# Krist-Marrakesh/Hybrid-Hotel-Recommendation-System-Based-on-Friends-Recommendations

Measured on AMD Instinct MI355X. Metric: fwd+bwd samples/sec (DCN-R train step) + scored (user,hotel) pairs/sec, higher is better.
Workload: dtype bf16; 1 GPU; DCN-R train step: fwd (train BN, dropout 0.6) + BCE + bwd + AdamW (+grad all-reduce), BASELINE configs[2]/[3]; batch_per_gpu=131072, global_batch=131072, tables=1M x 32 users, 100k x 32 hotels, 12 x 1000 x 32 cat, 8 dense, deep=3 cross + 4 x 512 residual, parallelism=dp1, exchange=none

## Files before the change

hybrid-hotel-recommendation-system-based-on-friends-recommendations_amd/csrc/dcnr_api.hip:

```cpp
#include "dcnr_internal.h"

#include <algorithm>
#include <cmath>
#include <cstdarg>
#include <cstdio>
#include <cstdlib>
#include <cstring>
#include <map>
#include <mutex>
#include <utility>
#include <vector>

namespace dcnr {

static thread_local char g_err[1024] = "";

void set_error(const char* fmt, ...) {
  va_list ap;
  va_start(ap, fmt);
  vsnprintf(g_err, sizeof(g_err), fmt, ap);
  va_end(ap);
}

dcnr_status set_max_dyn_lds(const void* kernel, size_t bytes) {
// ... 816 lines not shown
  return DCNR_OK;
}

dcnr_status linear_dx(const Dims& d, const void* X, const void* Wt, const void* R, void* C, int64_t B,
                      hipStream_t s) {
  GemmArgs g;
  memset(&g, 0, sizeof(g));
  g.A = X; g.lda = d.Hp; g.B = Wt; g.ldb = d.Hp; g.C = C; g.ldc = d.Hp;
  g.resid = R; g.ldr = R ? d.Hp : 0;
  g.M = B; g.N = d.Hp; g.K = d.Hp; g.k_per_split = d.Hp;
  TRYB(DCNR_K_GEMM_DX, s, (R ? 3 : 2) * act_b(d, B) + w_b(d, d.Hp),
       gemm_nn(d.prec, R ? EPI_STORE_RESID : EPI_STORE, g, 1, s));
  return DCNR_OK;
}

struct Fwd {
  const dcnr_model_desc* desc; const Dims& d; const Plan& pl; const Layout& L; const Params& P;
  const int64_t *user_ids, *item_ids, *cat_features; const float* num_features;
  int64_t B; float* logits; hipStream_t s; int check;
  GatherDesc g; CrossParams cp;
  const float* labels = nullptr; float grad_scale = 1.f; float* dz = nullptr;

  dcnr_status tower() const {
    TowerPack tp;
    memset(&tp, 0, sizeof(tp));
    tp.W0 = P.W0; tp.D = d.D; tp.b0 = P.b0;
    for (int j = 0; j < d.R; ++j) {
      const auto& Bk = P.blk[j];
      tp.w1[j] = Bk.w1; tp.b1[j] = Bk.b1; tp.g1[j] = Bk.g1; tp.be1[j] = Bk.be1; tp.rm1[j] = Bk.rm1; tp.rv1[j] = Bk.rv1;
      tp.w2[j] = Bk.w2; tp.b2[j] = Bk.b2; tp.g2[j] = Bk.g2; tp.be2[j] = Bk.be2; tp.rm2[j] = Bk.rm2; tp.rv2[j] = Bk.rv2;
    }
    tp.wf = P.wf; tp.H = d.H; tp.R = d.R; tp.out = L.twp; tp.err = check ? L.err : nullptr;
    TRYP(DCNR_K_PACK, s, tower_pack(tp, s));
    const GcOut o{nullptr, L.x0, L.zc, 0, d.Dp, nullptr};
    TRYB(DCNR_K_GATHER_CROSS, s, (double)B * (gather_row_b(d, desc->n_num) + (double)d.Dp * d.es + 4.0),
         gather_cross_out(g, cp, user_ids, item_ids, cat_features, num_features, B, o, 1, L.err, check, s));
// ... 3 lines not shown
    ta.wp = L.twp; ta.zc = L.zc; ta.bias = P.bf; ta.logits = logits; ta.err = L.err;
    ta.err_mirror = check ? desc->error_mirror : nullptr;
    TRYB(DCNR_K_TOWER, s, (double)B * (d.Dp * d.es + 8.0), eval_tower(ta, s));
    return DCNR_OK;
  }

  dcnr_status front(SideJoin& sj) const {
    const bool train = pl.train;
    if (train) {
      TRY(sj.fork(s));
      TRY(pack_all(d, P, L, train, sj.side));
      TRY(sj.mark());
    } else {
      TRY(pack_all(d, P, L, train, s, check != 0));
    }
    if (check && train) TRYP(DCNR_K_PACK, s, fill_zero(L.err, 4, s));
    if (train) {
      EmbBwdDesc eb;
      memset(&eb, 0, sizeof(eb));
      eb.n_tab = g.n_tab;
      for (int t = 0; t < g.n_tab; ++t) { eb.rows[t] = g.rows[t]; eb.width[t] = g.width[t]; }
      TRYB(DCNR_K_EMB_SORT, sj.side, 2.0 * 8.0 * g.n_tab * B + 8.0 * B * (2 + d.K) + 4.0 * B * 2,
           emb_sort(eb, user_ids, item_ids, cat_features, B, L.emb, sj.side));
      TRY(sj.record());
    }
    const GcOut o{nullptr, L.x0, L.zc, 0, d.Dp, train ? L.sc : nullptr};
    TRYB(DCNR_K_GATHER_CROSS, s, (double)B * (gather_row_b(d, desc->n_num) + (double)d.Dp * d.es + 4.0),
         gather_cross_out(g, cp, user_ids, item_ids, cat_features, num_features, B, o,
                          d.prec == DCNR_PREC_BF16, L.err, check, s));
    if (train) TRY(sj.wait_mark(s));
    TRYB(DCNR_K_GEMM_FWD, s, (double)B * d.Dp * d.es + act_b(d, B) + w_b(d, d.Dp),
// ... 192 lines not shown
      TRYB(DCNR_K_GEMM_DX, s, 5 * act_b(d, B) + w_b(d, d.Hp),
           linear_dx_bn(d, L, NT_EPI_RESID_SUM, da, L.W1t[j], du, L.G, nullptr, 0.f, nullptr, BnBufs{}, B,
                        &ncg, s, &xo1));
      TRY(dw1(j));
      TRY(bias_reduce(d, L, ncg, Gr.b0, accumulate, s, 2));
      b0_done = true;
    } else {
      TRY(linear_dx(d, dt1, L.W1t[j], du, L.G, B, s));
    }
    Gin = L.G;
    nc_du = 0;
    return DCNR_OK;
  }
};

struct BceOut { const float* labels; float grad_scale; float* loss; float* dlogits; double* part; };

dcnr_status forward_run(const dcnr_model_desc* desc, void* const* params,
                        const int64_t* user_ids, const int64_t* item_ids,
                        const int64_t* cat_features, const float* num_features, int64_t B,
                        int mode, uint64_t dropout_seed, float* logits, void* ws,
                        size_t ws_bytes, dcnr_stream_t stream, const BceOut* bce_out) {
  Dims d;
  TRY(make_dims(desc, &d));
  hipStream_t s = (hipStream_t)stream;
  if (!params || !logits || !ws || B < 0 || (B > 0 && (!user_ids || !item_ids)) ||
      (d.K > 0 && B > 0 && !cat_features) || (desc->n_num > 0 && B > 0 && !num_features)) {
    set_error("dcnr_forward: null argument");
    return DCNR_BAD_ARG;
  }
  if (mode == DCNR_TRAIN && B < 2) {
    set_error("Expected more than 1 value per channel when training");
    return DCNR_BAD_ARG;
  }
  const uint32_t flags = bce_out ? desc->flags : desc->flags & ~DCNR_FLAG_HEAD_STATS;
  const Plan pl = make_plan(d, flags, mode, B, desc->bn_allreduce != nullptr);
  const Layout L = make_layout(d, B, pl, ws);
  if (ws_bytes < L.total) {
    set_error("workspace too small: %zu < %zu", ws_bytes, L.total);
    return DCNR_WORKSPACE_TOO_SMALL;
  }
  if (B == 0) return DCNR_OK;
  const Params P = map_params(d, params);
  const int check = (desc->flags & DCNR_FLAG_CHECK_INDICES) ? 1 : 0;
  Fwd f{desc, d, pl, L, P, user_ids, item_ids, cat_features, num_features, B, logits, s, check,
        make_gather(d, P, desc->n_num), make_cross(d, P)};
  if (bce_out) { f.labels = bce_out->labels; f.grad_scale = bce_out->grad_scale; f.dz = bce_out->dlogits; }
  if (pl.tower) return f.tower();
  SideJoin sj;
  TRY(f.front(sj));
  TRY(pl.eval_epi ? f.eval_epi() : f.layers(dropout_seed));
  if (pl.train) TRY(sj.join(s));
  if (desc->error_mirror && check) TRYP(DCNR_K_PACK, s, mirror_word((const int*)ws, desc->error_mirror, s));
  if (bce_out)
    TRYP(DCNR_K_HEAD, s, bce(logits, bce_out->labels, B, bce_out->loss, pl.head_stats ? nullptr : bce_out->dlogits,
                             bce_out->grad_scale, bce_out->part, s));
  return DCNR_OK;
}


}
}

using namespace dcnr;

extern "C" {

int dcnr_abi_version(void) { return DCNR_ABI_VERSION; }
// ... 95 lines not shown
                             float* logits, float* loss, float* dlogits, void* bce_ws,
                             size_t bce_ws_bytes_, void* ws, size_t ws_bytes, dcnr_stream_t stream) {
  if (!labels || !loss || !dlogits || !bce_ws || B < 2) {
    set_error("dcnr_forward_bce: bad argument");
    return DCNR_BAD_ARG;
  }
  if (bce_ws_bytes_ < bce_ws_bytes()) {
    set_error("dcnr_forward_bce: loss workspace too small");
    return DCNR_WORKSPACE_TOO_SMALL;
  }
  const BceOut bo{labels, grad_scale, loss, dlogits, (double*)bce_ws};
  return forward_run(desc, params, user_ids, item_ids, cat_features, num_features, B, DCNR_TRAIN,
                     dropout_seed, logits, ws, ws_bytes, stream, &bo);
}

dcnr_status dcnr_backward(const dcnr_model_desc* desc, void* const* params, void* const* grads,
                          const int64_t* user_ids, const int64_t* item_ids,
                          const int64_t* cat_features, const float* num_features, int64_t B,
                          const float* dlogits, uint64_t dropout_seed, int accumulate, void* ws, size_t ws_bytes,
                          dcnr_stream_t stream) {
  Dims d;
  TRY(make_dims(desc, &d));
  hipStream_t s = (hipStream_t)stream;
  if (!params || !grads || !dlogits || !ws || B < 2) {
    set_error("dcnr_backward: bad argument");
    return DCNR_BAD_ARG;
  }
  const Plan pl = make_plan(d, desc->flags, DCNR_TRAIN, B, desc->bn_allreduce != nullptr);
  const Layout L = make_layout(d, B, pl, ws);
  if (ws_bytes < L.total) {
    set_error("workspace too small: %zu < %zu", ws_bytes, L.total);
    return DCNR_WORKSPACE_TOO_SMALL;
  }
  const Params P = map_params(d, params);
  const Grads Gr = map_grads(d, grads);
  const int Hp = d.Hp, H = d.H;
  if (pl.rowmap && accumulate) {
    set_error("dcnr_backward: DCNR_FLAG_ROW_MAP needs accumulate = 0");
    return DCNR_BAD_ARG;
  }
  if (pl.rowmap) {
    TRYB(DCNR_K_PACK, s, (double)L.rowmap_bytes, fill_zero(L.rowmap, L.rowmap_bytes, s));
  } else if (!accumulate) {
    void* zp[2 + MAX_CAT];
    int64_t zn[2 + MAX_CAT];
    for (int t = 0; t < 2 + d.K; ++t) { zp[t] = Gr.tab[t]; zn[t] = d.rows[t] * d.widths[t] * 4; }
    double zb = 0;
    for (int t = 0; t < 2 + d.K; ++t) zb += (double)zn[t];
    TRYB(DCNR_K_PACK, s, zb, fill_zero_multi(2 + d.K, zp, zn, s));
  }

  GatherDesc g = make_gather(d, P, desc->n_num);
  EmbBwdDesc eb;
  memset(&eb, 0, sizeof(eb));
  eb.n_tab = g.n_tab;
  eb.touched = L.rowmap;
  for (int t = 0; t < g.n_tab; ++t) {
    eb.grad[t] = Gr.tab[t]; eb.rows[t] = g.rows[t]; eb.width[t] = g.width[t]; eb.off[t] = g.off[t];
  }
  SideJoin sj;
  TRY(sj.fork(s));
  const CrossParams cpx = make_cross(d, P);
  CrossGrads cg;
  memset(&cg, 0, sizeof(cg));
  for (int l = 0; l < d.L; ++l) { cg.dw[l] = Gr.cw[l]; cg.db[l] = Gr.cb[l]; }
  cg.dwf_cross = Gr.wf + H;
  cg.dbf = Gr.bf;
  TRYB(DCNR_K_CROSS_BWD, sj.side, (double)B * (4.0 * (2 * d.L + 1) + 4.0 + 8.0 * (d.L + 1)) + (double)B * d.Dp * d.es,
       cross_backward(cpx, d.D, L.sc, dlogits, L.x0, d.prec == DCNR_PREC_BF16, d.Dp, B, cg, L.xcoef,
                      L.xalpha, L.cscratch, L.cscratch_bytes, accumulate, sj.side));
  TRY(sj.record());
  DwPipe dwp;
  DwPipe* pipe = nullptr;
  if (d.prec == DCNR_PREC_BF16 && (!g_prof || g_prof_mode == 2)) {
    TRY(dwp.init(sj.side, pl.dw_lag));
    pipe = &dwp;
  }

  Bwd c{desc, d, pl, L, P, Gr, B, dlogits, dropout_seed, accumulate, s, pipe};
  for (int j = d.R - 1; j >= 0; --j) TRY(pl.stats_epi ? c.block_epi(j, pl.xbn) : c.block_plain(j));
  TRY(linear_dw(d, L, L.G, Hp, Hp, L.x0, d.Dp, d.Dp, B, Gr.W0, H, d.D, accumulate, s, pipe));
  if (!c.b0_done) {
    int nc = 0;
    TRYB(DCNR_K_ROWWISE, s, act_b(d, B), col_sum(d.prec, L.G, B, Hp, Hp, L.part, &nc, s));
    TRY(bias_reduce(d, L, nc, Gr.b0, accumulate, s));
  }
  TRY(sj.join(s));
  if (desc->grad_ready) TRY(dwp.join(s));
  TRY(grads_ready(desc, DCNR_GRADS_DENSE, s));
  GemmArgs gx;
  memset(&gx, 0, sizeof(gx));
  gx.A = L.G; gx.lda = Hp; gx.B = L.W0t; gx.ldb = Hp; gx.C = L.dx0; gx.ldc = dq_of(d); gx.out_f32 = 1;
  gx.M = B; gx.N = d.Dp; gx.K = Hp; gx.k_per_split = Hp;
  TRYB(DCNR_K_GEMM_DX, s, act_b(d, B) + 4.0 * B * d.Dp + w_b(d, d.Dp), gemm_nn(d.prec, EPI_STORE, gx, 1, s));
  double ew = 0;
  for (int t = 0; t < 2 + d.K; ++t) ew += d.widths[t];
  eb.nv = d.L + 1;
  for (int l = 0; l < d.L; ++l) eb.V[l] = cpx.w[l];
  eb.V[d.L] = cpx.wf_cross;
  TRYB(DCNR_K_EMB_SUM, s, (double)B * (4.0 * ew + (8.0 + 4.0 * (d.L + 1)) * g.n_tab),
       emb_segment_sum(eb, L.emb, B, L.dx0, dq_of(d), L.xcoef, accumulate, s));
  if (!desc->grad_ready) TRY(dwp.join(s));
  TRY(grads_ready(desc, DCNR_GRADS_EMBEDDING, s));
  return DCNR_OK;
}

dcnr_status dcnr_gather_rows(const int64_t* idx, int64_t n, int64_t n_src, int32_t n_arrays,
                             const void* const* src, void* const* dst, const int64_t* row_bytes,
                             dcnr_stream_t stream) {
  hipStream_t s = (hipStream_t)stream;
  if (!src || !dst || !row_bytes || (n > 0 && !idx)) {
    set_error("dcnr_gather_rows: null argument");
    return DCNR_BAD_ARG;
  }
  TRYP(DCNR_K_SERVE, s, gather_rows(idx, n, n_src, n_arrays, src, dst, row_bytes, s));
  return DCNR_OK;
}

dcnr_status dcnr_candidate_union(const int64_t* positives, int64_t Q, const int64_t* knn_idx,
// ... 418 lines not shown
  TRYB(DCNR_K_ADAM, s, 28.0 * nparam, adam(n_tensors, params, grads, exp_avg, exp_avg_sq, numel, lr, beta1, beta2,
                         eps, weight_decay, step, decoupled, s));
  return DCNR_OK;
}

dcnr_status dcnr_adam_step_rows(int32_t n_tensors, float* const* params, const float* const* grads,
                                float* const* exp_avg, float* const* exp_avg_sq, const int64_t* numel,
                                const uint8_t* const* row_map, const int32_t* row_width,
                                float lr, float beta1, float beta2, float eps, float weight_decay,
                                int64_t step, int decoupled, dcnr_stream_t stream) {
  if (n_tensors < 0 || (n_tensors > 0 && (!params || !grads || !exp_avg || !exp_avg_sq || !numel ||
                                          !row_map || !row_width)) || step < 1) {
    set_error("dcnr_adam_step_rows: bad argument");
    return DCNR_BAD_ARG;
  }
  double nbytes = 0;
  for (int i = 0; i < n_tensors; ++i) {
    if (row_map[i] && (row_width[i] < 1 || numel[i] % row_width[i])) {
      set_error("dcnr_adam_step_rows: tensor %d: %lld elements in rows of %d", i, (long long)numel[i],
                row_width[i]);
      return DCNR_BAD_ARG;
    }
    nbytes += (row_map[i] ? 24.0 : 28.0) * (double)numel[i] +
              (row_map[i] ? (double)numel[i] / row_width[i] : 0.0);
  }
  hipStream_t s = (hipStream_t)stream;
  TRYB(DCNR_K_ADAM, s, nbytes, adam(n_tensors, params, grads, exp_avg, exp_avg_sq, numel, lr, beta1, beta2,
                                 eps, weight_decay, step, decoupled, s, row_map, row_width));
  return DCNR_OK;
}

dcnr_status dcnr_row_inv_norms(const float* table, int64_t N, int32_t d, float* inv_norms,
                               dcnr_stream_t stream) {
  if (!table || !inv_norms || d < 1 || N < 0) {
    set_error("dcnr_row_inv_norms: bad argument");
    return DCNR_BAD_ARG;
  }
  return row_inv_norms(table, N, d, inv_norms, (hipStream_t)stream);
}

size_t dcnr_cosine_topk_workspace_size(int64_t N, int64_t Q, int32_t k) {
  if (N < 1 || Q < 1 || k < 1) return 256;
  return topk_ws(N, Q, k) + 256;
}
// ... 241 lines not shown
```

hybrid-hotel-recommendation-system-based-on-friends-recommendations_amd/csrc/dcnr_internal.h:

```cpp
#pragma once
#include <hip/hip_runtime.h>
#include <hip/hip_ext.h>
#include <stdint.h>
#include <stddef.h>

#include <algorithm>
#include <cmath>

#include "../../include/dcnr.h"

namespace dcnr {

typedef __bf16 bf16;
typedef __attribute__((ext_vector_type(8))) __bf16 bf16x8;
typedef __attribute__((ext_vector_type(4))) __bf16 bf16x4;
typedef __attribute__((ext_vector_type(4))) short s16x4;
typedef __attribute__((ext_vector_type(4))) float f32x4;

constexpr int WAVE = 64;

void set_error(const char* fmt, ...);
dcnr_status set_max_dyn_lds(const void* kernel, size_t bytes);
#define DCNR_HIP(call)                                                              \
  do {                                                                              \
// ... 638 lines not shown
                              hipStream_t s);
dcnr_status requests_sources(const dcnr_interactions& store, const int32_t* reviewers,
                             const int32_t* modes, int64_t R, int64_t n_items,
                             const int64_t* pos_off, int64_t Q_total, int64_t* pos,
                             const int64_t* neg_off, int64_t neg_lo, int64_t neg_hi, int64_t* neg,
                             int32_t* counts, int32_t* status, int32_t* host_counts,
                             int32_t* host_status, hipStream_t s);
dcnr_status requests_recommended_by(const dcnr_interactions& store, const int32_t* reviewers,
                                    int64_t R, int64_t n_items, const int64_t* out_rows, int64_t n,
                                    const int64_t* offsets, const int32_t* out_count,
                                    const int64_t* list_off, int64_t L_total, int32_t* lists,
                                    int32_t* by_count, int64_t* by_off, int32_t* by_reviewers,
                                    int32_t* status, hipStream_t s);

dcnr_status fill_zero(void* p, size_t bytes, hipStream_t s);
dcnr_status mirror_word(const int* src, int* dst, hipStream_t s);
dcnr_status fill_zero_multi(int n, void* const* ptrs, const int64_t* bytes, hipStream_t s);

}
```

hybrid-hotel-recommendation-system-based-on-friends-recommendations_amd/csrc/elementwise.hip:

```cpp
#include "dcnr_internal.h"

#include <cmath>
#include <type_traits>

namespace dcnr {
namespace {

constexpr int NT = 256;
constexpr int UNROLL = 4;
constexpr int TARGET_CHUNKS = 2048;
constexpr int APPLY_CHUNKS = 8192;

template <typename T> constexpr int VE = 16 / (int)sizeof(T);

template <typename T>
__device__ __forceinline__ void ldv(const T* p, float (&o)[VE<T>]) {
  uint4 u = *reinterpret_cast<const uint4*>(p);
  if constexpr (std::is_same<T, float>::value) {
    o[0] = __uint_as_float(u.x); o[1] = __uint_as_float(u.y);
    o[2] = __uint_as_float(u.z); o[3] = __uint_as_float(u.w);
  } else {
    const bf16* h = reinterpret_cast<const bf16*>(&u);
#pragma unroll
    for (int i = 0; i < 8; ++i) o[i] = (float)h[i];
// ... 955 lines not shown
  const int vec_out = K % 4 == 0 && (uintptr_t)out % 16 == 0;
  hipLaunchKernelGGL(splitk_reduce_t_kernel, dim3((unsigned)cdiv(K, RT_K), (unsigned)cdiv(N, RT_N)),
                     dim3(256), 0, s, slab, splits, slab_stride, ld_slab, N, K, out, accumulate,
                     vec_out);
  DCNR_LAUNCH_CHECK();
  return DCNR_OK;
}

namespace {
__global__ __launch_bounds__(64) void zero_words_kernel(int* p, int n) {
  for (int i = threadIdx.x; i < n; i += 64) p[i] = 0;
}
__global__ __launch_bounds__(64) void mirror_word_kernel(const int* src, int* dst) {
  if (threadIdx.x == 0) __hip_atomic_store(dst, *src, __ATOMIC_RELAXED, __HIP_MEMORY_SCOPE_SYSTEM);
}
}

dcnr_status fill_zero(void* p, size_t bytes, hipStream_t s) {
  if (!bytes) return DCNR_OK;
  if (bytes <= 4096 && !(bytes & 3) && !((uintptr_t)p & 3)) {
    hipLaunchKernelGGL(zero_words_kernel, dim3(1), dim3(64), 0, s, (int*)p, (int)(bytes / 4));
    DCNR_LAUNCH_CHECK();
    return DCNR_OK;
  }
  DCNR_HIP(hipMemsetAsync(p, 0, bytes, s));
  return DCNR_OK;
}

dcnr_status mirror_word(const int* src, int* dst, hipStream_t s) {
  hipLaunchKernelGGL(mirror_word_kernel, dim3(1), dim3(64), 0, s, src, dst);
  DCNR_LAUNCH_CHECK();
  return DCNR_OK;
}

namespace {
constexpr int ZB_MAX = 66;
constexpr int ZB_CHUNK = NT * 16;
struct ZeroBatch {
  char* p[ZB_MAX]; int64_t bytes[ZB_MAX]; int64_t blk0[ZB_MAX + 1]; int n;
};
__global__ __launch_bounds__(NT) void zero_multi_kernel(ZeroBatch zb) {
  int t = 0;
  while (t + 1 < zb.n && (int64_t)blockIdx.x >= zb.blk0[t + 1]) ++t;
  char* p = zb.p[t];
  const int64_t n16 = zb.bytes[t] / 16;
// ... 37 lines not shown
```

hybrid-hotel-recommendation-system-based-on-friends-recommendations_amd/dcnr/_lib.py:

```python
from __future__ import annotations

import ctypes
import os
import threading

import torch

PKG_ROOT = os.path.dirname(os.path.dirname(os.path.abspath(__file__)))
LIB_PATH = os.environ.get("DCNR_LIB", os.path.join(PKG_ROOT, "lib", "libdcnr.so"))

DCNR_OK, DCNR_BAD_ARG, DCNR_INDEX_OOB, DCNR_HIP_ERROR, DCNR_UNSUPPORTED_SHAPE, \
    DCNR_WORKSPACE_TOO_SMALL = range(6)
PREC_FP32, PREC_BF16 = 0, 1
EVAL, TRAIN = 0, 1
FLAG_CHECK_INDICES = 1
FLAG_KEEP_INTERMEDIATES = 2
FLAG_FUSED_TOWER = 4
FLAG_ROW_MAP = 8
FLAG_HEAD_STATS = 16
ABI_VERSION = 4
WS_KINDS = ["x0", "h", "t1", "t2", "a1", "mask_a1", "mask_h", "bn_mean", "bn_invstd", "bn_scale",
            "bn_shift", "du", "dt2", "da", "dt1", "G", "dx0", "zc", "xcoef", "sc", "row_map"]

ALLREDUCE_FN = ctypes.CFUNCTYPE(ctypes.c_int, ctypes.c_void_p, ctypes.c_void_p, ctypes.c_int64,
# ... 25 lines not shown
    ]


class MetricsStruct(ctypes.Structure):
    _fields_ = [
        ("logloss", ctypes.c_double),
        ("auc", ctypes.c_double),
        ("rmse", ctypes.c_double),
        ("n", ctypes.c_int64),
        ("n_pos", ctypes.c_int64),
        ("n_neg", ctypes.c_int64),
        ("auc_u2", ctypes.c_int64),
        ("n_bad_label", ctypes.c_int64),
        ("n_nan", ctypes.c_int64),
    ]


class Interactions(ctypes.Structure):
    _fields_ = [
        ("n_reviewers", ctypes.c_int64),
        ("friend_offsets", ctypes.c_void_p),
        ("friend_rows", ctypes.c_void_p),
        ("n_friend_rows", ctypes.c_int64),
        ("review_offsets", ctypes.c_void_p),
        ("review_items", ctypes.c_void_p),
        ("review_rows", ctypes.c_void_p),
        ("n_reviews", ctypes.c_int64),
    ]


# ... 21 lines not shown
                                             _P, _P]),
    "dcnr_sparse_pack": (ctypes.c_int, [_P, _P, _I64, _P, ctypes.c_int32, ctypes.c_int32, _P, _P, _P]),
    "dcnr_sparse_accumulate": (ctypes.c_int, [_P, _I64, _I64, ctypes.c_int32, _P, _P, _P,
                                              ctypes.c_int32, _P]),
    "dcnr_bce_workspace_size": (ctypes.c_size_t, []),
    "dcnr_bce_with_logits": (ctypes.c_int, [_P, _P, _I64, _P, _P, ctypes.c_float, _P,
                                            ctypes.c_size_t, _P]),
    "dcnr_eval_metrics_workspace_size": (ctypes.c_size_t, [_I64]),
    "dcnr_eval_metrics": (ctypes.c_int, [_P, _P, _I64, _P, _P, ctypes.c_size_t, _P]),
    "dcnr_adam_step": (ctypes.c_int, [ctypes.c_int32, _P, _P, _P, _P, _P, ctypes.c_float,
                                      ctypes.c_float, ctypes.c_float, ctypes.c_float,
                                      ctypes.c_float, _I64, ctypes.c_int, _P]),
    "dcnr_adam_step_rows": (ctypes.c_int, [ctypes.c_int32, _P, _P, _P, _P, _P, _P, _P,
                                           ctypes.c_float, ctypes.c_float, ctypes.c_float,
                                           ctypes.c_float, ctypes.c_float, _I64, ctypes.c_int, _P]),
    "dcnr_row_inv_norms": (ctypes.c_int, [_P, _I64, ctypes.c_int32, _P, _P]),
    "dcnr_cosine_topk_workspace_size": (ctypes.c_size_t, [_I64, _I64, ctypes.c_int32]),
    "dcnr_cosine_topk": (ctypes.c_int, [_P, _P, _I64, ctypes.c_int32, _P, _I64, ctypes.c_int32,
                                        _P, _P, _P, ctypes.c_size_t, _P]),
    "dcnr_cosine_pack_rows": (ctypes.c_int, [_P, _P, _I64, ctypes.c_int32, _P, _P]),
    "dcnr_cosine_topk_packed": (ctypes.c_int, [_P, _P, _P, _I64, ctypes.c_int32, _P, _I64,
                                               ctypes.c_int32, _P, _P, _P, ctypes.c_size_t, _P]),
    "dcnr_cosine_neighbor_table_workspace_size": (ctypes.c_size_t, [_I64, ctypes.c_int32]),
    "dcnr_cosine_neighbor_table": (ctypes.c_int, [_P, _P, _P, _I64, ctypes.c_int32, ctypes.c_int32,
                                                  _I64, _I64, _P, _P, _P, ctypes.c_size_t, _P]),
    "dcnr_cosine_neighbor_table_update_workspace_size": (ctypes.c_size_t, [_I64, ctypes.c_int32,
                                                                           ctypes.c_int32, _I64]),
    "dcnr_cosine_neighbor_table_update": (ctypes.c_int, [_P, _P, _P, _I64, ctypes.c_int32,
                                                         ctypes.c_int32, _P, _I64, _P, _P, _P, _P, _P,
                                                         ctypes.c_size_t, _P]),
# ... 119 lines not shown
```

hybrid-hotel-recommendation-system-based-on-friends-recommendations_amd/dcnr/model.py:

```python
from __future__ import annotations

import ctypes
import threading
import time
from typing import Any, Dict, List, Optional

import numpy as np
import torch
import torch.nn as nn

from . import _lib


class CrossLayer(nn.Module):

    def __init__(self, input_dim):
        super().__init__()
        self.w = nn.Linear(input_dim, 1, bias=False)
        self.b = nn.Parameter(torch.zeros(input_dim))

    def forward(self, x):
        return x + x * self.w(x) + self.b


# ... 469 lines not shown
            model._index_watch.commit(slot, torch.cuda.current_stream(dev))
        else:
            model._index_watch.cancel(slot)
    _hook_error(model)
    _lib.check(st, call)
    if model.check_indices == "sync":
        _lib.check(lib.dcnr_check_errors(ws.data_ptr(), ws.numel(), _lib.stream_ptr(dev)),
                   "embedding")
    elif model.check_indices and slot is None and B > 0:
        model._index_watch.push(ws[:4])
    if bce is not None:
        return logits, ws, loss, dz
    return logits, ws


def run_backward(model: DCN_RecSys, user, item, cat, num, dlogits, ws, grads: List[torch.Tensor],
                 seed: int, accumulate=False, grad_ready=None, extra_flags: int = 0):
    lib = _lib.load()
    B = user.shape[0]
    desc = model.desc(grad_ready, extra_flags)
    model._active_ws = ws
    st = lib.dcnr_backward(ctypes.byref(desc), model.state_ptr_array(),
                           _lib.ptr_array(grads), user.data_ptr(), item.data_ptr(),
                           cat.data_ptr() if cat.numel() else None,
                           num.data_ptr() if num.numel() else None, B,
                           dlogits.data_ptr(), int(seed), 1 if accumulate else 0, ws.data_ptr(),
                           ws.numel(), _lib.stream_ptr(user.device))
    model._active_ws = None
    _hook_error(model)
    _lib.check(st, "dcnr_backward")
# ... 28 lines not shown
```

hybrid-hotel-recommendation-system-based-on-friends-recommendations_amd/dcnr/train.py:

```python
from __future__ import annotations

import ctypes
import math
from typing import Optional

import torch
import torch.distributed as dist

from . import _lib
from .model import DCN_RecSys, dropout_seed, run_backward, run_forward
from .ops import bce_with_logits


class PlateauLR:

    threshold = 1e-4
    eps = 1e-8

    def __init__(self, lr, patience=10, factor=0.1):
        if factor >= 1.0:
            raise ValueError("Factor should be < 1.0.")
        self.lr = float(lr)
        self.patience, self.factor = patience, factor
        self.best = math.inf
        self.num_bad_epochs = 0
# ... 76 lines not shown
        self._dense_work = None
        self._hook_error = None
        self._grad_ready_cb = _lib.GRAD_READY_FN(self._on_grads_ready) if self.world > 1 else None
        self.lr, self.wd, self.betas, self.eps = lr, weight_decay, betas, eps
        self.decoupled = optimizer_name == 'AdamW'
        self.step_count = 0
        self._ws = None
        self._grads = [p.grad for p in model.param_tensors()]
        self.row_map = self.world == 1 and not dense_table_grads
        self.dense_table_grads = dense_table_grads
        self._flags = _lib.FLAG_ROW_MAP if self.row_map else 0
        self.head_stats = bool(head_stats)
        if self.head_stats:
            self._flags |= _lib.FLAG_HEAD_STATS
        self._rows_cache = None
        self.step_events = None
        if sync_bn and self.world > 1:
            from .parallel import install_sync_bn
            install_sync_bn(model, process_group)

    def step(self, user, item, cat, num, y, return_logits=False):
        model = self.model
        model.train()
        user, item, cat, num = model.prepare_inputs(user, item, cat, num)
        y = y.reshape(-1).to(torch.float32).contiguous()
        seed = dropout_seed(user.device)
        model._index_watch.poll()
        sparse_rows = self._sparse_rows()
        flags = self._flags | (_lib.FLAG_ROW_MAP if sparse_rows else 0)
        if self.head_stats:
            logits, self._ws, loss, dz = run_forward(model, True, seed, user, item, cat, num,
                                                     self._ws, extra_flags=flags,
                                                     bce=(y, 1.0 / self.world))
        else:
            logits, self._ws = run_forward(model, True, seed, user, item, cat, num, self._ws,
                                           extra_flags=flags)
        self._B = user.shape[0]
        if self.exchange == "sparse" and self._sparse is not None:
            self._sparse.begin(self.touched_rows())
        if not self.head_stats:
            loss, dz = bce_with_logits(logits, y, True, 1.0 / self.world)
        self._dense_work = None
        if sparse_rows:
            lay = self._sparse_layout
# ... 17 lines not shown
        marks = self.step_events
        if marks is not None:
            e0 = torch.cuda.Event(enable_timing=True)
            e0.record()
        if self.row_map:
            self.step_count += 1
            self._adam_rows(self.step_count)
        else:
            self._exchange_and_update(None, None, dense)
        if marks is not None:
            e1 = torch.cuda.Event(enable_timing=True)
            e1.record()
            marks.append((e0, e1))
        return (loss, logits) if return_logits else loss

    def fit(self, train_loader, val, n_epochs=50, patience=5, lr_scheduler_patience=10,
            lr_scheduler_factor=0.1, checkpoint_path=None, on_epoch=None):
        if self.world > 1:
            raise NotImplementedError(
                "FusedTrainer.fit runs at world 1 only: a data-parallel epoch loop (sharded "
                "validation, one checkpoint writer) is not implemented; drive step() and "
                "dcnr.evaluate per rank instead")
        from .metrics import evaluate
        sched = PlateauLR(self.lr, patience=lr_scheduler_patience, factor=lr_scheduler_factor)
        history = {"epochs": [], "best_epoch": None, "best_val_loss": math.inf,
                   "stopped_early": False}
        no_improve = 0
        for epoch in range(n_epochs):
            for batch in train_loader:
                collab, cat, num, y = (t.to(self.flat.device) for t in batch)
# ... 186 lines not shown
```

include/dcnr.h:

```cpp
#ifndef DCNR_H
#define DCNR_H

#include <stddef.h>
#include <stdint.h>

#ifdef __cplusplus
extern "C" {
#endif

#define DCNR_ABI_VERSION 4

typedef void* dcnr_stream_t;

typedef enum {
  DCNR_OK = 0,
  DCNR_BAD_ARG = 1,
  DCNR_INDEX_OOB = 2,
  DCNR_HIP_ERROR = 3,
  DCNR_UNSUPPORTED_SHAPE = 4,
  DCNR_WORKSPACE_TOO_SMALL = 5
} dcnr_status;

typedef enum { DCNR_PREC_FP32 = 0, DCNR_PREC_BF16 = 1 } dcnr_precision;
typedef enum { DCNR_EVAL = 0, DCNR_TRAIN = 1 } dcnr_mode;
// ... 110 lines not shown

dcnr_status dcnr_eval_metrics(const float* logits, const float* labels, int64_t n,
                              dcnr_metrics* out, void* ws, size_t ws_bytes, dcnr_stream_t stream);

dcnr_status dcnr_adam_step(int32_t n_tensors, float* const* params, const float* const* grads,
                           float* const* exp_avg, float* const* exp_avg_sq, const int64_t* numel,
                           float lr, float beta1, float beta2, float eps, float weight_decay,
                           int64_t step, int decoupled, dcnr_stream_t stream);

dcnr_status dcnr_adam_step_rows(int32_t n_tensors, float* const* params, const float* const* grads,
                                float* const* exp_avg, float* const* exp_avg_sq, const int64_t* numel,
                                const uint8_t* const* row_map, const int32_t* row_width,
                                float lr, float beta1, float beta2, float eps, float weight_decay,
                                int64_t step, int decoupled, dcnr_stream_t stream);

dcnr_status dcnr_row_inv_norms(const float* table, int64_t N, int32_t d, float* inv_norms,
                               dcnr_stream_t stream);

size_t dcnr_cosine_topk_workspace_size(int64_t N, int64_t Q, int32_t k);

dcnr_status dcnr_cosine_topk(const float* table, const float* inv_norms, int64_t N, int32_t d,
                             const float* queries, int64_t Q, int32_t k, int64_t* idx,
                             float* dist, void* ws, size_t ws_bytes, dcnr_stream_t stream);

dcnr_status dcnr_cosine_pack_rows(const float* table, const float* inv_norms, int64_t N, int32_t d,
                                  uint16_t* packed, dcnr_stream_t stream);

dcnr_status dcnr_cosine_topk_packed(const float* table, const float* inv_norms, const uint16_t* packed,
                                    int64_t N, int32_t d, const float* queries, int64_t Q, int32_t k,
                                    int64_t* idx, float* dist, void* ws, size_t ws_bytes,
// ... 159 lines not shown
```

Baseline: 35.50 million samples/s.

## Fuse forward, loss, backward and row-wise Adam into one train-step call

Adds a single dcnr_train_step entry that runs forward, BCE, backward and the row-mapped AdamW update in one host call, and the trainer uses it when the configuration allows. The BCE loss, error-word mirroring and the rowmap zero-fill move onto the backward side stream so they overlap with dense backward work. The error word is cleared inside the mirror kernel, which lets the next step skip a separate zero-fill. The aim is to cut Python/ctypes dispatch and a few serialized small kernels per step, at the cost of extra cross-stream join bookkeeping and new state tracking for whether the workspace is clean.

```diff
diff --git a/hybrid-hotel-recommendation-system-based-on-friends-recommendations_amd/csrc/dcnr_api.hip b/hybrid-hotel-recommendation-system-based-on-friends-recommendations_amd/csrc/dcnr_api.hip
--- a/hybrid-hotel-recommendation-system-based-on-friends-recommendations_amd/csrc/dcnr_api.hip
+++ b/hybrid-hotel-recommendation-system-based-on-friends-recommendations_amd/csrc/dcnr_api.hip
@@ -854,12 +854,41 @@
   return DCNR_OK;
 }
 
+struct BceOut { const float* labels; float grad_scale; float* loss; float* dlogits; double* part; };
+
+dcnr_status adam_rows(const dcnr_adam_rows& o, hipStream_t s) {
+  double nbytes = 0;
+  for (int i = 0; i < o.n_tensors; ++i)
+    nbytes += (o.row_map[i] ? 24.0 : 28.0) * (double)o.numel[i] +
+              (o.row_map[i] ? (double)o.numel[i] / o.row_width[i] : 0.0);
+  TRYB(DCNR_K_ADAM, s, nbytes,
+       adam(o.n_tensors, o.params, o.grads, o.exp_avg, o.exp_avg_sq, o.numel, o.lr, o.beta1, o.beta2, o.eps,
+            o.weight_decay, o.step, o.decoupled, s, o.row_map, o.row_width));
+  return DCNR_OK;
+}
+
+struct StepSeams {
+  bool zero_err;
+  bool clear_err;
+  bool loss_side;
+  SideJoin* fwd_sj;
+  const BceOut* bce; const float* logits;
+  const dcnr_adam_rows* opt;
+};
+
+dcnr_status mirror_err(const dcnr_model_desc* desc, void* ws, bool clear, hipStream_t s) {
+  if (desc->error_mirror && (desc->flags & DCNR_FLAG_CHECK_INDICES))
+    TRYP(DCNR_K_PACK, s, mirror_word((int*)ws, desc->error_mirror, s, clear));
+  return DCNR_OK;
+}
+
 struct Fwd {
   const dcnr_model_desc* desc; const Dims& d; const Plan& pl; const Layout& L; const Params& P;
   const int64_t *user_ids, *item_ids, *cat_features; const float* num_features;
   int64_t B; float* logits; hipStream_t s; int check;
   GatherDesc g; CrossParams cp;
   const float* labels = nullptr; float grad_scale = 1.f; float* dz = nullptr;
+  bool zero_err = true;
 
   dcnr_status tower() const {
     TowerPack tp;
@@ -893,7 +922,7 @@
     } else {
       TRY(pack_all(d, P, L, train, s, check != 0));
     }
-    if (check && train) TRYP(DCNR_K_PACK, s, fill_zero(L.err, 4, s));
+    if (check && train && zero_err) TRYP(DCNR_K_PACK, s, fill_zero(L.err, 4, s));
     if (train) {
       EmbBwdDesc eb;
       memset(&eb, 0, sizeof(eb));
@@ -1116,13 +1145,12 @@
   }
 };
 
-struct BceOut { const float* labels; float grad_scale; float* loss; float* dlogits; double* part; };
-
 dcnr_status forward_run(const dcnr_model_desc* desc, void* const* params,
                         const int64_t* user_ids, const int64_t* item_ids,
                         const int64_t* cat_features, const float* num_features, int64_t B,
                         int mode, uint64_t dropout_seed, float* logits, void* ws,
-                        size_t ws_bytes, dcnr_stream_t stream, const BceOut* bce_out) {
+                        size_t ws_bytes, dcnr_stream_t stream, const BceOut* bce_out,
+                        const StepSeams* st = nullptr) {
   Dims d;
   TRY(make_dims(desc, &d));
   hipStream_t s = (hipStream_t)stream;
@@ -1149,11 +1177,14 @@
         make_gather(d, P, desc->n_num), make_cross(d, P)};
   if (bce_out) { f.labels = bce_out->labels; f.grad_scale = bce_out->grad_scale; f.dz = bce_out->dlogits; }
   if (pl.tower) return f.tower();
-  SideJoin sj;
+  if (st) f.zero_err = st->zero_err;
+  SideJoin own_sj;
+  SideJoin& sj = st && st->loss_side ? *st->fwd_sj : own_sj;
   TRY(f.front(sj));
   TRY(pl.eval_epi ? f.eval_epi() : f.layers(dropout_seed));
+  if (st && st->loss_side) return DCNR_OK;
   if (pl.train) TRY(sj.join(s));
-  if (desc->error_mirror && check) TRYP(DCNR_K_PACK, s, mirror_word((const int*)ws, desc->error_mirror, s));
+  TRY(mirror_err(desc, ws, st && st->clear_err, s));
   if (bce_out)
     TRYP(DCNR_K_HEAD, s, bce(logits, bce_out->labels, B, bce_out->loss, pl.head_stats ? nullptr : bce_out->dlogits,
                              bce_out->grad_scale, bce_out->part, s));
@@ -1279,11 +1310,9 @@
                      dropout_seed, logits, ws, ws_bytes, stream, &bo);
 }
 
-dcnr_status dcnr_backward(const dcnr_model_desc* desc, void* const* params, void* const* grads,
-                          const int64_t* user_ids, const int64_t* item_ids,
-                          const int64_t* cat_features, const float* num_features, int64_t B,
-                          const float* dlogits, uint64_t dropout_seed, int accumulate, void* ws, size_t ws_bytes,
-                          dcnr_stream_t stream) {
+static dcnr_status backward_run(const dcnr_model_desc* desc, void* const* params, void* const* grads,
+                                int64_t B, const float* dlogits, uint64_t dropout_seed, int accumulate,
+                                void* ws, size_t ws_bytes, dcnr_stream_t stream, const StepSeams* st) {
   Dims d;
   TRY(make_dims(desc, &d));
   hipStream_t s = (hipStream_t)stream;
@@ -1304,8 +1333,9 @@
     set_error("dcnr_backward: DCNR_FLAG_ROW_MAP needs accumulate = 0");
     return DCNR_BAD_ARG;
   }
+  const bool side_tail = st && st->loss_side;
   if (pl.rowmap) {
-    TRYB(DCNR_K_PACK, s, (double)L.rowmap_bytes, fill_zero(L.rowmap, L.rowmap_bytes, s));
+    if (!side_tail) TRYB(DCNR_K_PACK, s, (double)L.rowmap_bytes, fill_zero(L.rowmap, L.rowmap_bytes, s));
   } else if (!accumulate) {
     void* zp[2 + MAX_CAT];
     int64_t zn[2 + MAX_CAT];
@@ -1325,6 +1355,12 @@
   }
   SideJoin sj;
   TRY(sj.fork(s));
+  if (side_tail) {
+    TRY(mirror_err(desc, ws, st->clear_err, sj.side));
+    const BceOut& bo = *st->bce;
+    TRYP(DCNR_K_HEAD, sj.side, bce(st->logits, bo.labels, B, bo.loss, nullptr, bo.grad_scale, bo.part, sj.side));
+    TRYB(DCNR_K_PACK, sj.side, (double)L.rowmap_bytes, fill_zero(L.rowmap, L.rowmap_bytes, sj.side));
+  }
   const CrossParams cpx = make_cross(d, P);
   CrossGrads cg;
   memset(&cg, 0, sizeof(cg));
@@ -1351,6 +1387,7 @@
     TRY(bias_reduce(d, L, nc, Gr.b0, accumulate, s));
   }
   TRY(sj.join(s));
+  if (side_tail) st->fwd_sj->joined = true;
   if (desc->grad_ready) TRY(dwp.join(s));
   TRY(grads_ready(desc, DCNR_GRADS_DENSE, s));
   GemmArgs gx;
@@ -1367,7 +1404,64 @@
        emb_segment_sum(eb, L.emb, B, L.dx0, dq_of(d), L.xcoef, accumulate, s));
   if (!desc->grad_ready) TRY(dwp.join(s));
   TRY(grads_ready(desc, DCNR_GRADS_EMBEDDING, s));
-  return DCNR_OK;
+  if (st) TRY(adam_rows(*st->opt, s));
+  return DCNR_OK;
+}
+
+dcnr_status dcnr_backward(const dcnr_model_desc* desc, void* const* params, void* const* grads,
+                          const int64_t* user_ids, const int64_t* item_ids,
+                          const int64_t* cat_features, const float* num_features, int64_t B,
+                          const float* dlogits, uint64_t dropout_seed, int accumulate, void* ws, size_t ws_bytes,
+                          dcnr_stream_t stream) {
+  (void)user_ids; (void)item_ids; (void)cat_features; (void)num_features;
+  return backward_run(desc, params, grads, B, dlogits, dropout_seed, accumulate, ws, ws_bytes, stream, nullptr);
+}
+
+dcnr_status dcnr_train_step(const dcnr_model_desc* desc, void* const* params, void* const* grads,
+                            const int64_t* user_ids, const int64_t* item_ids,
+                            const int64_t* cat_features, const float* num_features, int64_t B,
+                            uint64_t dropout_seed, const float* labels, float grad_scale,
+                            float* logits, float* loss, float* dlogits, void* bce_ws,
+                            size_t bce_ws_bytes_, const dcnr_adam_rows* opt, int fresh_ws,
+                            uint32_t seams, void* ws, size_t ws_bytes, dcnr_stream_t stream) {
+  Dims d;
+  TRY(make_dims(desc, &d));
+  if (!params || !grads || !labels || !loss || !dlogits || !logits || !bce_ws || !ws || !opt || B < 2 ||
+      opt->n_tensors < 0 || opt->step < 1 ||
+      (opt->n_tensors > 0 && (!opt->params || !opt->grads || !opt->exp_avg || !opt->exp_avg_sq ||
+                              !opt->numel || !opt->row_map || !opt->row_width))) {
+    set_error("dcnr_train_step: bad argument");
+    return DCNR_BAD_ARG;
+  }
+  for (int i = 0; i < opt->n_tensors; ++i)
+    if (opt->row_map[i] && (opt->row_width[i] < 1 || opt->numel[i] % opt->row_width[i])) {
+      set_error("dcnr_train_step: tensor %d: %lld elements in rows of %d", i, (long long)opt->numel[i],
+                opt->row_width[i]);
+      return DCNR_BAD_ARG;
+    }
+  if (bce_ws_bytes_ < bce_ws_bytes()) {
+    set_error("dcnr_train_step: loss workspace too small");
+    return DCNR_WORKSPACE_TOO_SMALL;
+  }
+  const Plan pl = make_plan(d, desc->flags, DCNR_TRAIN, B, desc->bn_allreduce != nullptr);
+  if (!pl.head_stats || !pl.rowmap || desc->grad_ready || desc->bn_allreduce) {
+    set_error("dcnr_train_step: needs DCNR_FLAG_ROW_MAP, an applicable DCNR_FLAG_HEAD_STATS and no hooks");
+    return DCNR_UNSUPPORTED_SHAPE;
+  }
+  const bool check = (desc->flags & DCNR_FLAG_CHECK_INDICES) != 0;
+  const BceOut bo{labels, grad_scale, loss, dlogits, (double*)bce_ws};
+  SideJoin fwd_sj;
+  StepSeams st{};
+  st.clear_err = (seams & DCNR_STEP_ERR_WORD) && check && desc->error_mirror;
+  st.zero_err = !(seams & DCNR_STEP_ERR_WORD) || fresh_ws;
+  st.loss_side = (seams & DCNR_STEP_LOSS_SIDE) && !(g_prof && g_prof_mode == 1);
+  st.fwd_sj = &fwd_sj;
+  st.bce = &bo;
+  st.logits = logits;
+  st.opt = opt;
+  TRY(forward_run(desc, params, user_ids, item_ids, cat_features, num_features, B, DCNR_TRAIN, dropout_seed,
+                  logits, ws, ws_bytes, stream, &bo, &st));
+  return backward_run(desc, params, grads, B, dlogits, dropout_seed, 0, ws, ws_bytes, stream, &st);
 }
 
 dcnr_status dcnr_gather_rows(const int64_t* idx, int64_t n, int64_t n_src, int32_t n_arrays,
@@ -1816,20 +1910,15 @@
     set_error("dcnr_adam_step_rows: bad argument");
     return DCNR_BAD_ARG;
   }
-  double nbytes = 0;
-  for (int i = 0; i < n_tensors; ++i) {
+  for (int i = 0; i < n_tensors; ++i)
     if (row_map[i] && (row_width[i] < 1 || numel[i] % row_width[i])) {
       set_error("dcnr_adam_step_rows: tensor %d: %lld elements in rows of %d", i, (long long)numel[i],
                 row_width[i]);
       return DCNR_BAD_ARG;
     }
-    nbytes += (row_map[i] ? 24.0 : 28.0) * (double)numel[i] +
-              (row_map[i] ? (double)numel[i] / row_width[i] : 0.0);
-  }
-  hipStream_t s = (hipStream_t)stream;
-  TRYB(DCNR_K_ADAM, s, nbytes, adam(n_tensors, params, grads, exp_avg, exp_avg_sq, numel, lr, beta1, beta2,
-                                 eps, weight_decay, step, decoupled, s, row_map, row_width));
-  return DCNR_OK;
+  const dcnr_adam_rows o{n_tensors, params, grads, exp_avg, exp_avg_sq, numel, row_map, row_width,
+                         lr, beta1, beta2, eps, weight_decay, step, decoupled};
+  return adam_rows(o, (hipStream_t)stream);
 }
 
 dcnr_status dcnr_row_inv_norms(const float* table, int64_t N, int32_t d, float* inv_norms,
diff --git a/hybrid-hotel-recommendation-system-based-on-friends-recommendations_amd/csrc/dcnr_internal.h b/hybrid-hotel-recommendation-system-based-on-friends-recommendations_amd/csrc/dcnr_internal.h
--- a/hybrid-hotel-recommendation-system-based-on-friends-recommendations_amd/csrc/dcnr_internal.h
+++ b/hybrid-hotel-recommendation-system-based-on-friends-recommendations_amd/csrc/dcnr_internal.h
@@ -676,7 +676,7 @@
                                     int32_t* status, hipStream_t s);
 
 dcnr_status fill_zero(void* p, size_t bytes, hipStream_t s);
-dcnr_status mirror_word(const int* src, int* dst, hipStream_t s);
+dcnr_status mirror_word(int* src, int* dst, hipStream_t s, bool clear = false);
 dcnr_status fill_zero_multi(int n, void* const* ptrs, const int64_t* bytes, hipStream_t s);
 
 }
diff --git a/hybrid-hotel-recommendation-system-based-on-friends-recommendations_amd/csrc/elementwise.hip b/hybrid-hotel-recommendation-system-based-on-friends-recommendations_amd/csrc/elementwise.hip
--- a/hybrid-hotel-recommendation-system-based-on-friends-recommendations_amd/csrc/elementwise.hip
+++ b/hybrid-hotel-recommendation-system-based-on-friends-recommendations_amd/csrc/elementwise.hip
@@ -993,6 +993,12 @@
 __global__ __launch_bounds__(64) void mirror_word_kernel(const int* src, int* dst) {
   if (threadIdx.x == 0) __hip_atomic_store(dst, *src, __ATOMIC_RELAXED, __HIP_MEMORY_SCOPE_SYSTEM);
 }
+__global__ __launch_bounds__(64) void mirror_clear_word_kernel(int* src, int* dst) {
+  if (threadIdx.x == 0) {
+    __hip_atomic_store(dst, *src, __ATOMIC_RELAXED, __HIP_MEMORY_SCOPE_SYSTEM);
+    *src = 0;
+  }
+}
 }
 
 dcnr_status fill_zero(void* p, size_t bytes, hipStream_t s) {
@@ -1006,8 +1012,9 @@
   return DCNR_OK;
 }
 
-dcnr_status mirror_word(const int* src, int* dst, hipStream_t s) {
-  hipLaunchKernelGGL(mirror_word_kernel, dim3(1), dim3(64), 0, s, src, dst);
+dcnr_status mirror_word(int* src, int* dst, hipStream_t s, bool clear) {
+  if (clear) hipLaunchKernelGGL(mirror_clear_word_kernel, dim3(1), dim3(64), 0, s, src, dst);
+  else hipLaunchKernelGGL(mirror_word_kernel, dim3(1), dim3(64), 0, s, (const int*)src, dst);
   DCNR_LAUNCH_CHECK();
   return DCNR_OK;
 }
diff --git a/hybrid-hotel-recommendation-system-based-on-friends-recommendations_amd/dcnr/_lib.py b/hybrid-hotel-recommendation-system-based-on-friends-recommendations_amd/dcnr/_lib.py
--- a/hybrid-hotel-recommendation-system-based-on-friends-recommendations_amd/dcnr/_lib.py
+++ b/hybrid-hotel-recommendation-system-based-on-friends-recommendations_amd/dcnr/_lib.py
@@ -63,6 +63,29 @@
         ("n_bad_label", ctypes.c_int64),
         ("n_nan", ctypes.c_int64),
     ]
+
+
+class AdamRows(ctypes.Structure):
+    _fields_ = [
+        ("n_tensors", ctypes.c_int32),
+        ("params", ctypes.c_void_p),
+        ("grads", ctypes.c_void_p),
+        ("exp_avg", ctypes.c_void_p),
+        ("exp_avg_sq", ctypes.c_void_p),
+        ("numel", ctypes.c_void_p),
+        ("row_map", ctypes.c_void_p),
+        ("row_width", ctypes.c_void_p),
+        ("lr", ctypes.c_float),
+        ("beta1", ctypes.c_float),
+        ("beta2", ctypes.c_float),
+        ("eps", ctypes.c_float),
+        ("weight_decay", ctypes.c_float),
+        ("step", ctypes.c_int64),
+        ("decoupled", ctypes.c_int32),
+    ]
+
+
+STEP_ERR_WORD, STEP_LOSS_SIDE, STEP_ALL = 1, 2, 3
 
 
 class Interactions(ctypes.Structure):
@@ -114,6 +137,10 @@
     "dcnr_adam_step_rows": (ctypes.c_int, [ctypes.c_int32, _P, _P, _P, _P, _P, _P, _P,
                                            ctypes.c_float, ctypes.c_float, ctypes.c_float,
                                            ctypes.c_float, ctypes.c_float, _I64, ctypes.c_int, _P]),
+    "dcnr_train_step": (ctypes.c_int, [ctypes.POINTER(ModelDesc), _P, _P, _P, _P, _P, _P, _I64,
+                                       ctypes.c_uint64, _P, ctypes.c_float, _P, _P, _P, _P,
+                                       ctypes.c_size_t, ctypes.POINTER(AdamRows), ctypes.c_int,
+                                       ctypes.c_uint32, _P, ctypes.c_size_t, _P]),
     "dcnr_row_inv_norms": (ctypes.c_int, [_P, _I64, ctypes.c_int32, _P, _P]),
     "dcnr_cosine_topk_workspace_size": (ctypes.c_size_t, [_I64, _I64, ctypes.c_int32]),
     "dcnr_cosine_topk": (ctypes.c_int, [_P, _P, _I64, ctypes.c_int32, _P, _I64, ctypes.c_int32,
diff --git a/hybrid-hotel-recommendation-system-based-on-friends-recommendations_amd/dcnr/model.py b/hybrid-hotel-recommendation-system-based-on-friends-recommendations_amd/dcnr/model.py
--- a/hybrid-hotel-recommendation-system-based-on-friends-recommendations_amd/dcnr/model.py
+++ b/hybrid-hotel-recommendation-system-based-on-friends-recommendations_amd/dcnr/model.py
@@ -507,6 +507,46 @@
     return logits, ws
 
 
+def run_train_step(model: DCN_RecSys, seed: int, user, item, cat, num, y, grad_scale: float,
+                   ws: torch.Tensor, ws_clean: bool, grads: List[torch.Tensor], opt,
+                   extra_flags: int, seams: int = _lib.STEP_ALL):
+    lib = _lib.load()
+    B = user.shape[0]
+    dev = user.device
+    logits = torch.empty(B, dtype=torch.float32, device=dev)
+    loss = torch.empty((), dtype=torch.float32, device=dev)
+    dz = torch.empty(B, dtype=torch.float32, device=dev)
+    lws = torch.empty(int(lib.dcnr_bce_workspace_size()), dtype=torch.uint8, device=dev)
+    state = model.state_ptr_array()
+    desc = model.desc(extra_flags=extra_flags)
+    slot = None
+    if model.check_indices and model.check_indices != "sync":
+        slot, mirror = model._index_watch.reserve()
+        if slot is not None:
+            desc.error_mirror = mirror
+    model._active_ws = ws
+    st = lib.dcnr_train_step(ctypes.byref(desc), state, _lib.ptr_array(grads), user.data_ptr(),
+                             item.data_ptr(), cat.data_ptr() if cat.numel() else None,
+                             num.data_ptr() if num.numel() else None, B, seed, y.data_ptr(),
+                             float(grad_scale), logits.data_ptr(), loss.data_ptr(), dz.data_ptr(),
+                             lws.data_ptr(), lws.numel(), ctypes.byref(opt), 0 if ws_clean else 1,
+                             int(seams), ws.data_ptr(), ws.numel(), _lib.stream_ptr(dev))
+    model._active_ws = None
+    if slot is not None:
+        if st == 0:
+            model._index_watch.commit(slot, torch.cuda.current_stream(dev))
+        else:
+            model._index_watch.cancel(slot)
+    if st == _lib.DCNR_UNSUPPORTED_SHAPE and \
+            (lib.dcnr_last_error() or b"").startswith(b"dcnr_train_step: needs"):
+        return None
+    _lib.check(st, "dcnr_train_step")
+    if model.check_indices and slot is None:
+        model._index_watch.push(ws[:4])
+    clean = bool(seams & _lib.STEP_ERR_WORD) and slot is not None
+    return logits, loss, dz, clean
+
+
 def run_backward(model: DCN_RecSys, user, item, cat, num, dlogits, ws, grads: List[torch.Tensor],
                  seed: int, accumulate=False, grad_ready=None, extra_flags: int = 0):
     lib = _lib.load()
diff --git a/hybrid-hotel-recommendation-system-based-on-friends-recommendations_amd/dcnr/train.py b/hybrid-hotel-recommendation-system-based-on-friends-recommendations_amd/dcnr/train.py
--- a/hybrid-hotel-recommendation-system-based-on-friends-recommendations_amd/dcnr/train.py
+++ b/hybrid-hotel-recommendation-system-based-on-friends-recommendations_amd/dcnr/train.py
@@ -8,7 +8,7 @@
 import torch.distributed as dist
 
 from . import _lib
-from .model import DCN_RecSys, dropout_seed, run_backward, run_forward
+from .model import DCN_RecSys, dropout_seed, run_backward, run_forward, run_train_step
 from .ops import bce_with_logits
 
 
@@ -115,6 +115,10 @@
         if self.head_stats:
             self._flags |= _lib.FLAG_HEAD_STATS
         self._rows_cache = None
+        self.seams = _lib.STEP_ALL
+        self.last_step_one_call = False
+        self._ws_clean = False
+        self._one_call_refused = None
         self.step_events = None
         if sync_bn and self.world > 1:
             from .parallel import install_sync_bn
@@ -129,6 +133,13 @@
         model._index_watch.poll()
         sparse_rows = self._sparse_rows()
         flags = self._flags | (_lib.FLAG_ROW_MAP if sparse_rows else 0)
+        if self._one_call_wanted():
+            out = self._step_one_call(user, item, cat, num, y, seed, flags)
+            if out is not None:
+                loss, logits = out
+                return (loss, logits) if return_logits else loss
+        self.last_step_one_call = False
+        self._ws_clean = False
         if self.head_stats:
             logits, self._ws, loss, dz = run_forward(model, True, seed, user, item, cat, num,
                                                      self._ws, extra_flags=flags,
@@ -176,6 +187,39 @@
             marks.append((e0, e1))
         return (loss, logits) if return_logits else loss
 
+    def _one_call_wanted(self):
+        model = self.model
+        return (self.seams and self.world == 1 and self.row_map and self.head_stats
+                and self._grad_ready_cb is None and model.bn_allreduce is None
+                and self.step_events is None and model.check_indices != "sync"
+                and self._one_call_refused != (model.precision, model.keep_intermediates))
+
+    def _step_one_call(self, user, item, cat, num, y, seed, flags):
+        model = self.model
+        B = user.shape[0]
+        nbytes = model.workspace_bytes(B, _lib.TRAIN, flags)
+        if self._ws is None or self._ws.numel() < nbytes:
+            self._ws = torch.empty(nbytes, dtype=torch.uint8, device=user.device)
+            self._ws_clean = False
+        self._B = B
+        p, g, m, v, numel, maps, widths, n = self._row_segments()
+        cast = lambda a: ctypes.cast(a, ctypes.c_void_p)
+        opt = _lib.AdamRows(n, cast(p), cast(g), cast(m), cast(v), cast(numel), cast(maps),
+                            cast(widths), float(self.lr), float(self.betas[0]), float(self.betas[1]),
+                            float(self.eps), float(self.wd), self.step_count + 1,
+                            1 if self.decoupled else 0)
+        clean, self._ws_clean = self._ws_clean, False
+        out = run_train_step(model, seed, user, item, cat, num, y, 1.0 / self.world, self._ws, clean,
+                             self._grads, opt, flags, self.seams)
+        if out is None:
+            self._one_call_refused = (model.precision, model.keep_intermediates)
+            return None
+        logits, loss, _, self._ws_clean = out
+        self.step_count += 1
+        self._dense_work = None
+        self.last_step_one_call = True
+        return loss, logits
+
     def fit(self, train_loader, val, n_epochs=50, patience=5, lr_scheduler_patience=10,
             lr_scheduler_factor=0.1, checkpoint_path=None, on_epoch=None):
         if self.world > 1:
diff --git a/include/dcnr.h b/include/dcnr.h
--- a/include/dcnr.h
+++ b/include/dcnr.h
@@ -148,6 +148,32 @@
                                 float lr, float beta1, float beta2, float eps, float weight_decay,
                                 int64_t step, int decoupled, dcnr_stream_t stream);
 
+typedef struct {
+  int32_t n_tensors;
+  float* const* params;
+  const float* const* grads;
+  float* const* exp_avg;
+  float* const* exp_avg_sq;
+  const int64_t* numel;
+  const uint8_t* const* row_map;
+  const int32_t* row_width;
+  float lr, beta1, beta2, eps, weight_decay;
+  int64_t step;
+  int32_t decoupled;
+} dcnr_adam_rows;
+
+#define DCNR_STEP_ERR_WORD 1u
+#define DCNR_STEP_LOSS_SIDE 2u
+#define DCNR_STEP_ALL 3u
+
+dcnr_status dcnr_train_step(const dcnr_model_desc* desc, void* const* params, void* const* grads,
+                            const int64_t* user_ids, const int64_t* item_ids,
+                            const int64_t* cat_features, const float* num_features, int64_t B,
+                            uint64_t dropout_seed, const float* labels, float grad_scale,
+                            float* logits, float* loss, float* dlogits, void* bce_ws,
+                            size_t bce_ws_bytes, const dcnr_adam_rows* opt, int fresh_ws,
+                            uint32_t seams, void* ws, size_t ws_bytes, dcnr_stream_t stream);
+
 dcnr_status dcnr_row_inv_norms(const float* table, int64_t N, int32_t d, float* inv_norms,
                                dcnr_stream_t stream);
 
```

New measurement: 35.32 million samples/s. Within noise of the previous version (-0.5%).
